# Yuer867/EMO-Disentanger

Hardware: AMD Instinct MI355X
Metric: train tokens/sec (+ AR gen tokens/sec in "gen"), stage2 Performer d512 L12 seq2048 (higher is better)
Workload: dtype bf16; 1 GPU; BASELINE configs[1]: stage2 Performer d_model=512 n_layer=12 n_head=8 favor_dims=128 seq=2048, B=64/GPU, dropout 0.1, omega redraw every_forward, fwd+bwd+allreduce+clip+Adam; global_batch=64, seq_len=2048, parallelism=dp1

## Files before the change

emo-disentanger_amd/csrc/emo_gemm_w128.hip:

```cpp
#include "emo_gemm_epi.h"

namespace {
constexpr int W_BM = 256, W_BN = 256, W_BK = 64;
constexpr int W_TILE = 256 * W_BK * 2;
constexpr int W_NA = 3, W_NB = 2;
constexpr int W_LDS = (W_NA + W_NB) * W_TILE;

__device__ __forceinline__ uint32_t w_lds_addr(const void* p) { return (uint32_t)(uintptr_t)(const __attribute__((address_space(3))) char*)p; }

__device__ __forceinline__ void w_dma2(const char* sbase, uint32_t o0, uint32_t o1, uint32_t lds_dst) {
    uint32_t keep;
    asm volatile("s_mov_b32 %0, m0\n\ts_mov_b32 m0, %4\n\ts_nop 0\n\tglobal_load_lds_dwordx4 %1, %3\n\ts_add_u32 m0, m0, 0x400\n\ts_nop 0\n\t"
                 "global_load_lds_dwordx4 %2, %3\n\ts_mov_b32 m0, %0"
                 : "=&s"(keep) : "v"(o0), "v"(o1), "s"(sbase), "s"(lds_dst) : "memory", "scc");
}
__device__ __forceinline__ void w_dma2_nt(const char* sbase, uint32_t o0, uint32_t o1, uint32_t lds_dst) {
    uint32_t keep;
    asm volatile("s_mov_b32 %0, m0\n\ts_mov_b32 m0, %4\n\ts_nop 0\n\tglobal_load_lds_dwordx4 %1, %3 nt\n\ts_add_u32 m0, m0, 0x400\n\ts_nop 0\n\t"
                 "global_load_lds_dwordx4 %2, %3 nt\n\ts_mov_b32 m0, %0"
                 : "=&s"(keep) : "v"(o0), "v"(o1), "s"(sbase), "s"(lds_dst) : "memory", "scc");
}
__device__ __forceinline__ void w_mma(f32x4& c, const bf16x8& a, const bf16x8& b) {
    asm volatile("v_mfma_f32_16x16x32_bf16 %0, %1, %2, %0" : "+a"(c) : "v"(a), "v"(b));
}
__device__ __forceinline__ void w_mma_v(f32x4& c, const bf16x8& a, const bf16x8& b) {
    asm volatile("s_nop 3\n\tv_mfma_f32_16x16x32_bf16 %0, %1, %2, %0" : "+v"(c) : "v"(a), "v"(b));
}
__device__ __forceinline__ void w_mma_drain() { asm volatile("s_nop 15\n\ts_nop 15" ::: "memory"); }
__device__ __forceinline__ void w_drop8(const DropCtx& d, uint64_t idx0, float (&v)[8]) {
    const uint32_t lo = (uint32_t)(idx0 >> 2), hi = (uint32_t)(idx0 >> 34) * 0x9E3779B1u;
#pragma unroll
    for (int q = 0; q < 2; ++q) {
        const uint32_t h = emo_drop_hash(d, (lo + q) ^ hi), h2 = emo_xs32(h);
        v[4 * q] *= (h & 0xFFFFu) >= d.thr16 ? d.scale : 0.f;
        v[4 * q + 1] *= (h >> 16) >= d.thr16 ? d.scale : 0.f;
        v[4 * q + 2] *= (h2 & 0xFFFFu) >= d.thr16 ? d.scale : 0.f;
        v[4 * q + 3] *= (h2 >> 16) >= d.thr16 ? d.scale : 0.f;
    }
}
template <int N> __device__ __forceinline__ void w_wait();
template <> __device__ __forceinline__ void w_wait<0>() { asm volatile("s_waitcnt vmcnt(0)" ::: "memory"); }
template <> __device__ __forceinline__ void w_wait<8>() { asm volatile("s_waitcnt vmcnt(8)" ::: "memory"); }
template <> __device__ __forceinline__ void w_wait<24>() { asm volatile("s_waitcnt vmcnt(24)" ::: "memory"); }

template <typename OutT>
__global__ __launch_bounds__(256, 1) void gemm_w128_kernel(const bf16_t* __restrict__ A, int64_t lda, const bf16_t* __restrict__ B, int64_t ldb,
                                                          OutT* __restrict__ C, int64_t M, int64_t N, int64_t K, EpiParams ep) {
    extern __shared__ __attribute__((aligned(16))) char smem[];
#ifdef EMO_DIAG
    const uint64_t dg_t0 = __builtin_readcyclecounter();
    uint64_t dg_sync = 0, dg_loop0 = 0, dg_loop1 = 0;
#endif
    const int tid = threadIdx.x, lane = tid & 63;
    const int wave = __builtin_amdgcn_readfirstlane(tid >> 6);
    const int wr = wave >> 1, wc = wave & 1;
    const int64_t tiles_n = N / W_BN, tiles_m = M / W_BM;
    const int64_t bid = blockIdx.x, xcd = bid & 7, local = bid >> 3;
    const int64_t tn = local % tiles_n, tm = (local / tiles_n) * 8 + xcd;
    if (tm >= tiles_m) return;
    const int64_t m0 = tm * W_BM, n0 = tn * W_BN;
    const int nk = (int)(K / W_BK);

    uint32_t offA[8], offB[8];
#pragma unroll
    for (int i = 0; i < 8; ++i) {
        const int r = (wave * 8 + i) * 8 + (lane >> 3);
        offA[i] = (uint32_t)((r * lda + ((lane & 7) ^ (r & 7)) * 8) * 2);
        offB[i] = (uint32_t)((r * ldb + ((lane & 7) ^ (((r >> 1) & 1) | (((r >> 3) & 3) << 1))) * 8) * 2);
    }
    const char* gA = (const char*)(A + m0 * lda);
    const char* gB = (const char*)(B + n0 * ldb);
    const uint32_t lds0 = __builtin_amdgcn_readfirstlane(w_lds_addr(smem));
    const uint32_t dstw = lds0 + wave * 8192;
    const uint32_t foA = (uint32_t)((lane & 15) * 128 + ((((lane >> 4)) ^ (lane & 7)) << 4)) + wr * 128 * 128;
    const uint32_t foB = (uint32_t)((8 * ((lane & 15) >> 2) + (lane & 3)) * 128 + (((lane >> 4) ^ (((lane >> 1) & 1) | (((lane >> 2) & 3) << 1))) << 4)) +
                         W_NA * W_TILE + wc * 128 * 128;

    f32x4 acc[8][8];
#pragma unroll
    for (int i = 0; i < 8; ++i)
#pragma unroll
        for (int j = 0; j < 8; ++j) acc[i][j] = (f32x4){0.f, 0.f, 0.f, 0.f};

    int sa_issue = 0, sb_issue = 0;
    int t_issueA = 0, t_issueB = 0;
    const bool a_nt = ep.a_nt != 0;
    auto issueA_part = [&](int g) {
        if (a_nt) w_dma2_nt(gA + (int64_t)t_issueA * (W_BK * 2), offA[2 * g], offA[2 * g + 1], dstw + sa_issue * W_TILE + g * 2048);
        else w_dma2(gA + (int64_t)t_issueA * (W_BK * 2), offA[2 * g], offA[2 * g + 1], dstw + sa_issue * W_TILE + g * 2048);
    };
    auto issueB_part = [&](int g) { w_dma2(gB + (int64_t)t_issueB * (W_BK * 2), offB[2 * g], offB[2 * g + 1], dstw + (W_NA + sb_issue) * W_TILE + g * 2048); };
    auto doneA = [&]() { ++t_issueA; sa_issue = sa_issue == W_NA - 1 ? 0 : sa_issue + 1; };
    auto doneB = [&]() { ++t_issueB; sb_issue ^= 1; };
#pragma unroll
    for (int s = 0; s < 5; ++s) {
        const bool isA = (s & 1) == 0;
#pragma unroll
        for (int g = 0; g < 4; ++g) { if (isA) issueA_part(g); else issueB_part(g); }
        if (isA) { doneA(); if (t_issueA > nk - 1) t_issueA = nk - 1; } else { doneB(); if (t_issueB > nk - 1) t_issueB = nk - 1; }
    }
    w_wait<24>();
    __builtin_amdgcn_s_barrier();
    asm volatile("" ::: "memory");

    bf16x8 fa[2][8], fb[2][8];
    int sa = 0, sb = 0;
    const char* ldsb = smem;
    auto rd = [&](int set, int q, uint32_t a_off, uint32_t b_off) {
        if (q < 8) fb[set][q] = *(const bf16x8*)(ldsb + b_off + (32 * (q >> 1) + 4 * (q & 1)) * 128);
        else fa[set][q - 8] = *(const bf16x8*)(ldsb + a_off + (q - 8) * 2048);
    };
    {
        const uint32_t a_off = foA, b_off = foB;
#pragma unroll
        for (int q = 0; q < 16; ++q) rd(0, q, a_off, b_off);
    }
    constexpr int RQ[9] = {0, 3, 6, 9, 12, 14, 16, 16, 16};
#ifdef EMO_DIAG
    dg_loop0 = __builtin_readcyclecounter();
#endif
    for (int t = 0; t < nk; ++t) {
        const uint32_t a_off = (foA + sa * W_TILE) ^ 64u, b_off = (foB + sb * W_TILE) ^ 64u;
#pragma unroll
        for (int i = 0; i < 8; ++i) {
#pragma unroll
            for (int q = RQ[i]; q < RQ[i + 1]; ++q) rd(1, q, a_off, b_off);
#pragma unroll
            for (int j = 0; j < 8; ++j) w_mma(acc[i][j], fb[0][j], fa[0][i]);
            __builtin_amdgcn_sched_barrier(0);
        }
#ifdef EMO_DIAG
        const uint64_t dg_s0 = __builtin_readcyclecounter();
#endif
        asm volatile("s_waitcnt lgkmcnt(0)" ::: "memory");
        w_wait<8>();
        __builtin_amdgcn_s_barrier();
        asm volatile("" ::: "memory");
#ifdef EMO_DIAG
        dg_sync += __builtin_readcyclecounter() - dg_s0;
#endif
        sa = sa == W_NA - 1 ? 0 : sa + 1;
        sb ^= 1;
        const uint32_t a_nx = foA + sa * W_TILE, b_nx = foB + sb * W_TILE;
#pragma unroll
        for (int i = 0; i < 8; ++i) {
#pragma unroll
            for (int q = RQ[i]; q < RQ[i + 1]; ++q) rd(0, q, a_nx, b_nx);
            if (i < 4) issueB_part(i); else issueA_part(i - 4);
#pragma unroll
            for (int j = 0; j < 8; ++j) w_mma(acc[i][j], fb[1][j], fa[1][i]);
            __builtin_amdgcn_sched_barrier(0);
        }
        doneB(); if (t_issueB > nk - 1) t_issueB = nk - 1;
        doneA(); if (t_issueA > nk - 1) t_issueA = nk - 1;
    }
#ifdef EMO_DIAG
    dg_loop1 = __builtin_readcyclecounter();
#endif
    w_wait<0>();
    w_mma_drain();
    const int ecol = 8 * (lane >> 4);
    {
        f32x4 bv[4][2];
#pragma unroll
        for (int h = 0; h < 4; ++h)
#pragma unroll
            for (int q = 0; q < 2; ++q) bv[h][q] = ep.bias ? *(const f32x4*)(ep.bias + n0 + wc * 128 + 32 * h + ecol + 4 * q) : (f32x4){0.f, 0.f, 0.f, 0.f};
        const OutT* rp = (const OutT*)ep.residual;
#pragma clang loop unroll(full)
        for (int i2 = 0; i2 < 4; ++i2) {
            bf16x8 res[2][4];
            if (rp) {
#pragma unroll
                for (int u = 0; u < 2; ++u)
#pragma unroll
                    for (int h = 0; h < 4; ++h)
                        res[u][h] = *(const bf16x8*)(rp + (m0 + wr * 128 + (2 * i2 + u) * 16 + (lane & 15)) * ep.ldc + n0 + wc * 128 + 32 * h + ecol);
            }
#pragma clang loop unroll(full)
            for (int u = 0; u < 2; ++u) {
                const int i = 2 * i2 + u;
                const int64_t m = m0 + wr * 128 + i * 16 + (lane & 15);
#pragma clang loop unroll(full)
                for (int h = 0; h < 4; ++h) {
                    const int64_t n = n0 + wc * 128 + 32 * h + ecol;
                    float v[8];
#pragma unroll
                    for (int r = 0; r < 4; ++r) { v[r] = acc[i][2 * h][r] + bv[h][0][r]; v[4 + r] = acc[i][2 * h + 1][r] + bv[h][1][r]; }
                    if (ep.drop.thr16) w_drop8(ep.drop, (uint64_t)(m * N + n), v);
                    if (rp) {
#pragma unroll
                        for (int r = 0; r < 8; ++r) v[r] += (float)res[u][h][r];
                    }
                    bf16x8 o;
#pragma unroll
                    for (int r = 0; r < 8; ++r) o[r] = (bf16_t)v[r];
                    if (ep.nt_store) __builtin_nontemporal_store(o, (bf16x8*)(C + m * ep.ldc + n));
                    else *(bf16x8*)(C + m * ep.ldc + n) = o;
                }
            }
        }
    }
#ifdef EMO_DIAG
    if (ep.ablate == 8 && ep.rln_stats && lane == 0) {
        unsigned long long* dg = (unsigned long long*)ep.rln_stats;
        const uint64_t t1 = __builtin_readcyclecounter();
        atomicAdd(dg + 0, (unsigned long long)(dg_loop0 - dg_t0));
        atomicAdd(dg + 1, (unsigned long long)(dg_loop1 - dg_loop0));
        atomicAdd(dg + 2, (unsigned long long)dg_sync);
        atomicAdd(dg + 3, (unsigned long long)(t1 - dg_loop1));
        atomicAdd(dg + 4, 1ull);
    }
#endif
}

__device__ __forceinline__ int w_swz_k(int k) { return (k & 3) | (((k >> 3) & 1) << 2); }

template <int RS>
__global__ __launch_bounds__(256, 1) void gemm_w128_tn_kernel(const bf16_t* __restrict__ A, int64_t lda, const bf16_t* __restrict__ B, int64_t ldb,
                                                             float* __restrict__ Cws, int64_t M, int64_t N, int64_t K, int64_t kps, float* __restrict__ a_rowsum, float* __restrict__ b_rowsum,
                                                             int full, int extra, int nt_mask, float* __restrict__ rs_ws) {
    extern __shared__ __attribute__((aligned(16))) char smem[];
    const int tid = threadIdx.x, lane = tid & 63;
    const int wave = __builtin_amdgcn_readfirstlane(tid >> 6);
    const int wr = wave >> 1, wc = wave & 1;
    const int64_t tiles_n = N / W_BN, ntile = (M / W_BM) * tiles_n;
    const int64_t bid = blockIdx.x, xcd = bid & 7, q = bid >> 3;
    int64_t split, t_id;
    if (q < (int64_t)full * ntile) { split = xcd * full + q / ntile; t_id = q % ntile; }
    else {
        const int64_t left = 32 - (int64_t)full * ntile, slot = xcd * left + (q - (int64_t)full * ntile);
        if (slot >= (int64_t)extra * ntile) return;
        split = 8 * full + slot / ntile;
        t_id = slot % ntile;
    }
    const int64_t tm = t_id / tiles_n, tn = t_id % tiles_n;
    const int64_t m0 = tm * W_BM, n0 = tn * W_BN;
    const int64_t kbeg = split * kps;
    const int64_t kend = (kbeg + kps < K) ? kbeg + kps : K;
    float* C = Cws + split * M * N;
    const int nk = kbeg < kend ? (int)((kend - kbeg) / W_BK) : 0;
    if (nk == 0) {
#pragma unroll 4
        for (int e = tid; e < 256 * 64; e += 256) *(f32x4*)(C + (m0 + (e >> 6)) * N + n0 + (e & 63) * 4) = (f32x4){0.f, 0.f, 0.f, 0.f};
        if (RS == 1 && rs_ws) rs_ws[(split * tiles_n + tn) * M + m0 + tid] = 0.f;
        if (RS == 2 && rs_ws) rs_ws[(split * (M / W_BM) + tm) * N + n0 + tid] = 0.f;
        return;
    }
    uint32_t offA[8], offB[8];
#pragma unroll
    for (int i = 0; i < 8; ++i) {
        const int J = wave * 8 + i, half = J >> 4, j = J & 15;
        const int k = j * 4 + (lane >> 4), p16 = lane & 15, g = (p16 >> 1) ^ w_swz_k(k);
        offA[i] = (uint32_t)((k * lda + half * 128 + (g * 2 + (p16 & 1)) * 8) * 2);
        offB[i] = (uint32_t)((k * ldb + half * 128 + (g * 2 + (p16 & 1)) * 8) * 2);
    }
    const char* gA = (const char*)(A + kbeg * lda + m0);
    const char* gB = (const char*)(B + kbeg * ldb + n0);
    const int64_t stepA = 64 * lda * 2, stepB = 64 * ldb * 2;
    const uint32_t lds0 = __builtin_amdgcn_readfirstlane(w_lds_addr(smem));
    const uint32_t dstw = lds0 + wave * 8192;
    const int li = lane & 15;
    const uint32_t fo = (uint32_t)((((lane >> 4) * 8 + (li >> 2)) * 256) | ((((li >> 2) & 3) | (((lane >> 4) & 1) << 2)) << 5) | ((li & 3) << 3));
    const uint32_t foA = fo + wr * 16384, foB = fo + W_NA * W_TILE + wc * 16384;

    f32x4 acc[8][8];
#pragma unroll
    for (int i = 0; i < 8; ++i)
#pragma unroll
        for (int j = 0; j < 8; ++j) acc[i][j] = (f32x4){0.f, 0.f, 0.f, 0.f};
    f32x4 rs[4];
#pragma unroll
    for (int u = 0; u < 4; ++u) rs[u] = (f32x4){0.f, 0.f, 0.f, 0.f};
    const bf16_t one_b = (bf16_t)1.f;
    bf16x8 ones = {one_b, one_b, one_b, one_b, one_b, one_b, one_b, one_b};
    asm volatile("" : "+v"(ones));
    const int rs_mod = RS == 2 ? (int)(M / W_BM) : (int)tiles_n, rs_me = RS == 2 ? (int)tm : (int)tn;
    int rs_phase = RS ? (int)((kbeg / W_BK) % rs_mod) : 0;

    int sa_issue = 0, sb_issue = 0, t_issueA = 0, t_issueB = 0;
    const bool a_nt = (nt_mask & 1) != 0, b_nt = (nt_mask & 2) != 0;
    auto issueA_part = [&](int g) {
        if (a_nt) w_dma2_nt(gA + (int64_t)t_issueA * stepA, offA[2 * g], offA[2 * g + 1], dstw + sa_issue * W_TILE + g * 2048);
        else w_dma2(gA + (int64_t)t_issueA * stepA, offA[2 * g], offA[2 * g + 1], dstw + sa_issue * W_TILE + g * 2048);
    };
    auto issueB_part = [&](int g) {
        if (b_nt) w_dma2_nt(gB + (int64_t)t_issueB * stepB, offB[2 * g], offB[2 * g + 1], dstw + (W_NA + sb_issue) * W_TILE + g * 2048);
        else w_dma2(gB + (int64_t)t_issueB * stepB, offB[2 * g], offB[2 * g + 1], dstw + (W_NA + sb_issue) * W_TILE + g * 2048);
    };
    auto doneA = [&]() { ++t_issueA; sa_issue = sa_issue == W_NA - 1 ? 0 : sa_issue + 1; if (t_issueA > nk - 1) t_issueA = nk - 1; };
    auto doneB = [&]() { ++t_issueB; sb_issue ^= 1; if (t_issueB > nk - 1) t_issueB = nk - 1; };
#pragma unroll
    for (int s = 0; s < 5; ++s) {
        const bool isA = (s & 1) == 0;
#pragma unroll
        for (int g = 0; g < 4; ++g) { if (isA) issueA_part(g); else issueB_part(g); }
        if (isA) doneA(); else doneB();
    }
    w_wait<24>();
    __builtin_amdgcn_s_barrier();
    asm volatile("" ::: "memory");

    bf16x8 fa[2][8], fb[2][8];
    int sa = 0, sb = 0;
    const char* ldsb = smem;
    auto rd1 = [&](uint32_t off) -> bf16x8 {
        bf16x8 v;
#pragma unroll
        for (int h = 0; h < 2; ++h) {
            const short4v t = __builtin_amdgcn_ds_read_tr16_b64_v4i16((__attribute__((address_space(3))) short4v*)(ldsb + off + h * 1024));
            const bf16x4 tb = __builtin_bit_cast(bf16x4, t);
            v[4 * h] = tb[0]; v[4 * h + 1] = tb[1]; v[4 * h + 2] = tb[2]; v[4 * h + 3] = tb[3];
        }
        return v;
    };
    auto rd = [&](int set, int q2, uint32_t a_off, uint32_t b_off, int ks8) {
        if (q2 < 8) fb[set][q2] = rd1((b_off ^ (uint32_t)(q2 << 5)) + ks8);
        else fa[set][q2 - 8] = rd1((a_off ^ (uint32_t)((q2 - 8) << 5)) + ks8);
    };
#pragma unroll
    for (int q2 = 0; q2 < 16; ++q2) rd(0, q2, foA, foB, 0);
    constexpr int RQ[9] = {0, 3, 6, 9, 12, 14, 16, 16, 16};
    for (int t = 0; t < nk; ++t) {
        const uint32_t a_off = foA + sa * W_TILE, b_off = foB + sb * W_TILE;
        const bool rs_on = RS && rs_phase == rs_me;
#pragma unroll
        for (int i = 0; i < 8; ++i) {
#pragma unroll
            for (int q2 = RQ[i]; q2 < RQ[i + 1]; ++q2) rd(1, q2, a_off, b_off, 8192);
#pragma unroll
            for (int j = 0; j < 8; ++j) w_mma(acc[i][j], fb[0][j], fa[0][i]);
            if (RS == 1 && rs_on && (i & 1) == wc) w_mma_v(rs[i >> 1], ones, fa[0][i]);
            if (RS == 2 && rs_on && (i & 1) == wr) w_mma_v(rs[i >> 1], fb[0][i], ones);
            __builtin_amdgcn_sched_barrier(0);
        }
        asm volatile("s_waitcnt lgkmcnt(0)" ::: "memory");
        w_wait<8>();
        __builtin_amdgcn_s_barrier();
        asm volatile("" ::: "memory");
        sa = sa == W_NA - 1 ? 0 : sa + 1;
        sb ^= 1;
        const uint32_t a_nx = foA + sa * W_TILE, b_nx = foB + sb * W_TILE;
#pragma unroll
        for (int i = 0; i < 8; ++i) {
#pragma unroll
            for (int q2 = RQ[i]; q2 < RQ[i + 1]; ++q2) rd(0, q2, a_nx, b_nx, 0);
            if (i < 4) issueB_part(i); else issueA_part(i - 4);
#pragma unroll
            for (int j = 0; j < 8; ++j) w_mma(acc[i][j], fb[1][j], fa[1][i]);
            if (RS == 1 && rs_on && (i & 1) == wc) w_mma_v(rs[i >> 1], ones, fa[1][i]);
            if (RS == 2 && rs_on && (i & 1) == wr) w_mma_v(rs[i >> 1], fb[1][i], ones);
            __builtin_amdgcn_sched_barrier(0);
        }
        doneB();
        doneA();
        if (RS) { if (++rs_phase == rs_mod) rs_phase = 0; }
    }
    w_wait<0>();
    w_mma_drain();
    if (RS == 1 && (lane >> 4) == 0) {
        float* dst = rs_ws ? rs_ws + (split * tiles_n + tn) * M : nullptr;
#pragma unroll
        for (int u = 0; u < 4; ++u) {
            const int64_t m = m0 + wr * 128 + (2 * u + wc) * 16 + lane;
            if (dst) dst[m] = rs[u][0]; else atomicAdd(a_rowsum + m, rs[u][0]);
        }
    }
    if (RS == 2 && (lane & 15) == 0) {
        float* dst = rs_ws ? rs_ws + (split * (M / W_BM) + tm) * N : nullptr;
#pragma unroll
        for (int u = 0; u < 4; ++u) {
            const int64_t n = n0 + wc * 128 + (2 * u + wr) * 16 + (lane >> 4) * 4;
            if (dst) *(f32x4*)(dst + n) = rs[u];
            else {
#pragma unroll
                for (int r = 0; r < 4; ++r) atomicAdd(b_rowsum + n + r, rs[u][r]);
            }
        }
    }
#pragma clang loop unroll(full)
    for (int i = 0; i < 8; ++i) {
        float* crow = C + (m0 + wr * 128 + i * 16 + (lane & 15)) * N + n0 + wc * 128 + (lane >> 4) * 4;
#pragma clang loop unroll(full)
        for (int j = 0; j < 8; ++j) *(f32x4*)(crow + j * 16) = acc[i][j];
    }
}
}

bool emo_gemm_w128_try(const bf16_t* A, int64_t lda, const bf16_t* B, int64_t ldb, void* C, int dtype_out, int64_t M, int64_t N, int64_t K,
                       const EpiParams& ep, hipStream_t st) {
    const char* e = getenv("EMO_GEMM_W128");
    const int mode = e ? atoi(e) : -1;
    if (mode == 0) return false;
    if ((M % W_BM) || (N % W_BN) || (K % W_BK) || K < 4 * W_BK || dtype_out != EMO_BF16) return false;
    if (mode < 0 && (K < 1024 || (M / W_BM) * (N / W_BN) < 256)) return false;
    if (ep.atomic || ep.accumulate || ep.ws_stride || ep.a_rowsum || ep.b_rowsum || ep.ln_c1 || ep.rln_x || ep.mask_out) return false;
    if (ep.aux_out || ep.mul_mode != EMO_MUL_NONE || ep.act != EMO_ACT_NONE) return false;
    if ((lda & 7) || (ldb & 7) || (ep.ldc & 7) || (((uintptr_t)A | (uintptr_t)B | (uintptr_t)C) & 15)) return false;
    if ((uint64_t)(256 * (lda > ldb ? lda : ldb) + 64) * 2 >= 0xFFFF0000ull) return false;
    const int64_t tiles_m = M / W_BM, tiles_n = N / W_BN;
    dim3 grid((unsigned)(((tiles_m + 7) / 8) * 8 * tiles_n));
    EpiParams ep2 = ep;
    { const char* e4 = getenv("EMO_W128_NT_STORE"); ep2.nt_store = e4 ? atoi(e4) : 0; }
    { const char* e3 = getenv("EMO_W128_A_NT"); ep2.a_nt = e3 ? atoi(e3) : 1; }
    auto k = gemm_w128_kernel<bf16_t>;
    static bool attr = false;
    if (!attr) { (void)hipFuncSetAttribute((const void*)k, hipFuncAttributeMaxDynamicSharedMemorySize, W_LDS); attr = true; }
    hipLaunchKernelGGL(k, grid, dim3(256), W_LDS, st, A, lda, B, ldb, (bf16_t*)C, M, N, K, ep2);
    return true;
}

static int64_t w_tn_plan(int64_t M, int64_t N, int64_t K, int& full, int& extra) {
    full = extra = 0;
    const char* e = getenv("EMO_GEMM_W128");
    if (e && atoi(e) == 0) return 0;
    const char* e2 = getenv("EMO_GEMM_W128_TN");
    if (e2 && atoi(e2) == 0) return 0;
    if ((M % W_BM) || (N % W_BN) || (K % W_BK)) return 0;
    const int64_t ntile = (M / W_BM) * (N / W_BN), nkt = K / W_BK;
    if (ntile > 32) return 0;
    int64_t f = 32 / ntile;
    if (f > 8) f = 8;
    int64_t x = f < 8 ? (8 * (32 - f * ntile)) / ntile : 0;
    if (e2 && atoi(e2) == 2) x = 0;
    int64_t min_kt = 16;
    { const char* e3 = getenv("EMO_W128_TN_MINKT"); if (e3 && atoi(e3) > 0) min_kt = atoi(e3); }
    while (nkt / (8 * f + x) < min_kt) {
        if (x) x = 0;
        else if (f > 1) --f;
        else return 0;
    }
    int64_t min_blk = 96;
    { const char* e4 = getenv("EMO_W128_TN_MINBLK"); if (e4 && atoi(e4) > 0) min_blk = atoi(e4); }
    if (ntile * (8 * f + x) < min_blk) return 0;
    full = (int)f;
    extra = (int)x;
    return 8 * f + x;
}
int64_t emo_gemm_w128_tn_splits(int64_t M, int64_t N, int64_t K) {
    int full, extra;
    return w_tn_plan(M, N, K, full, extra);
}

void emo_splitk_reduce_launch(const float* ws, int64_t stride, int splits, float* out, int64_t n4, int accumulate, hipStream_t st);
void emo_splitk_reduce_rs_launch(const float* ws, int64_t stride, int splits, float* out, int64_t n4, int accumulate, const float* rs_ws, int64_t rs_stride,
                                 int rs_parts, float* rs_out, hipStream_t st);
int64_t emo_gemm_w128_tn_rs_floats(int64_t M, int64_t N, int64_t splits) {
    const int64_t a = (N / W_BN) * M, b = (M / W_BM) * N;
    return splits * (a > b ? a : b);
}

bool emo_gemm_w128_tn_try(const bf16_t* A, int64_t lda, const bf16_t* B, int64_t ldb, float* C, int64_t ldc, int64_t M, int64_t N, int64_t K, int accumulate,
                          float* a_rowsum, float* b_rowsum, void* ws, int64_t ws_bytes, hipStream_t st) {
    int full, extra;
    const int64_t splits0 = w_tn_plan(M, N, K, full, extra);
    if (!splits0 || ldc != N || !ws || ((uintptr_t)ws & 15) || ws_bytes < splits0 * M * N * (int64_t)sizeof(float)) return false;
    if ((lda & 7) || (ldb & 7) || (((uintptr_t)A | (uintptr_t)B | (uintptr_t)C) & 15)) return false;
    if ((uint64_t)(64 * (lda > ldb ? lda : ldb) + 256) * 2 >= 0xFFFF0000ull) return false;
    const int64_t kps = ((K / W_BK + splits0 - 1) / splits0) * W_BK;
    const int64_t ntile = (M / W_BM) * (N / W_BN);
    dim3 grid(256);
    int nt_mask = 0;
    { const char* e3 = getenv("EMO_W128_TN_NT"); if (e3) nt_mask = atoi(e3); }
    float* rs_ws = nullptr;
    if ((a_rowsum || b_rowsum) && ws_bytes >= (splits0 * M * N + emo_gemm_w128_tn_rs_floats(M, N, splits0)) * (int64_t)sizeof(float) &&
        !(((uintptr_t)a_rowsum | (uintptr_t)b_rowsum) & 15))
        rs_ws = (float*)ws + splits0 * M * N;
#define W_TN_LAUNCH(RSv)                                                                                                                     \
    do {                                                                                                                                     \
        auto k = gemm_w128_tn_kernel<RSv>;                                                                                                   \
        static bool attr = false;                                                                                                            \
        if (!attr) { (void)hipFuncSetAttribute((const void*)k, hipFuncAttributeMaxDynamicSharedMemorySize, W_LDS); attr = true; }            \
        hipLaunchKernelGGL(k, grid, dim3(256), W_LDS, st, A, lda, B, ldb, (float*)ws, M, N, K, kps, a_rowsum, b_rowsum, full, extra, nt_mask, rs_ws); \
    } while (0)
    if (a_rowsum) W_TN_LAUNCH(1); else if (b_rowsum) W_TN_LAUNCH(2); else W_TN_LAUNCH(0);
#undef W_TN_LAUNCH
    if (rs_ws)
        emo_splitk_reduce_rs_launch((const float*)ws, M * N, (int)splits0, C, (M * N) >> 2, accumulate, rs_ws, a_rowsum ? M : N,
                                    (int)(splits0 * (a_rowsum ? N / W_BN : M / W_BM)), a_rowsum ? a_rowsum : b_rowsum, st);
    else
        emo_splitk_reduce_launch((const float*)ws, M * N, (int)splits0, C, (M * N) >> 2, accumulate, st);
    return true;
}
```

Baseline: 2.971 million tokens/s.

## Add 8-wave variant of split-K TN weight-gradient GEMM kernel

Adds a 512-thread (8-wave) version of the 256x256 split-K TN GEMM kernel. Each wave now owns a 128x64 sub-tile instead of 128x128, with per-wave DMA slices and wait counts adjusted to match. Higher-priority scheduling is set on the upper four waves. This becomes the default path, with an env var to fall back to the 4-wave kernel. The aim is more latency hiding and better MFMA/LDS overlap per CU. In exchange each wave does more LDS reads relative to its MFMA work.

```diff
diff --git a/emo-disentanger_amd/csrc/emo_gemm_w128.hip b/emo-disentanger_amd/csrc/emo_gemm_w128.hip
--- a/emo-disentanger_amd/csrc/emo_gemm_w128.hip
+++ b/emo-disentanger_amd/csrc/emo_gemm_w128.hip
@@ -40,7 +40,9 @@
 }
 template <int N> __device__ __forceinline__ void w_wait();
 template <> __device__ __forceinline__ void w_wait<0>() { asm volatile("s_waitcnt vmcnt(0)" ::: "memory"); }
+template <> __device__ __forceinline__ void w_wait<4>() { asm volatile("s_waitcnt vmcnt(4)" ::: "memory"); }
 template <> __device__ __forceinline__ void w_wait<8>() { asm volatile("s_waitcnt vmcnt(8)" ::: "memory"); }
+template <> __device__ __forceinline__ void w_wait<12>() { asm volatile("s_waitcnt vmcnt(12)" ::: "memory"); }
 template <> __device__ __forceinline__ void w_wait<24>() { asm volatile("s_waitcnt vmcnt(24)" ::: "memory"); }
 
 template <typename OutT>
@@ -384,6 +386,178 @@
 #pragma clang loop unroll(full)
         for (int j = 0; j < 8; ++j) *(f32x4*)(crow + j * 16) = acc[i][j];
     }
+}
+
+namespace w8 {
+template <int RS>
+__global__ __launch_bounds__(512, 1) void gemm_w128_tn_kernel(const bf16_t* __restrict__ A, int64_t lda, const bf16_t* __restrict__ B, int64_t ldb,
+                                                             float* __restrict__ Cws, int64_t M, int64_t N, int64_t K, int64_t kps, float* __restrict__ a_rowsum, float* __restrict__ b_rowsum,
+                                                             int full, int extra, int nt_mask, float* __restrict__ rs_ws) {
+    extern __shared__ __attribute__((aligned(16))) char smem[];
+    const int tid = threadIdx.x, lane = tid & 63;
+    const int wave = __builtin_amdgcn_readfirstlane(tid >> 6);
+    const int wm = wave >> 2, wn = wave & 3;
+    const int64_t tiles_n = N / W_BN, ntile = (M / W_BM) * tiles_n;
+    const int64_t bid = blockIdx.x, xcd = bid & 7, q = bid >> 3;
+    int64_t split, t_id;
+    if (q < (int64_t)full * ntile) { split = xcd * full + q / ntile; t_id = q % ntile; }
+    else {
+        const int64_t left = 32 - (int64_t)full * ntile, slot = xcd * left + (q - (int64_t)full * ntile);
+        if (slot >= (int64_t)extra * ntile) return;
+        split = 8 * full + slot / ntile;
+        t_id = slot % ntile;
+    }
+    const int64_t tm = t_id / tiles_n, tn = t_id % tiles_n;
+    const int64_t m0 = tm * W_BM, n0 = tn * W_BN;
+    const int64_t kbeg = split * kps;
+    const int64_t kend = (kbeg + kps < K) ? kbeg + kps : K;
+    float* C = Cws + split * M * N;
+    const int nk = kbeg < kend ? (int)((kend - kbeg) / W_BK) : 0;
+    if (nk == 0) {
+#pragma unroll 4
+        for (int e = tid; e < 256 * 64; e += 512) *(f32x4*)(C + (m0 + (e >> 6)) * N + n0 + (e & 63) * 4) = (f32x4){0.f, 0.f, 0.f, 0.f};
+        if (RS == 1 && rs_ws && tid < 256) rs_ws[(split * tiles_n + tn) * M + m0 + tid] = 0.f;
+        if (RS == 2 && rs_ws && tid < 256) rs_ws[(split * (M / W_BM) + tm) * N + n0 + tid] = 0.f;
+        return;
+    }
+    uint32_t offA[4], offB[4];
+#pragma unroll
+    for (int i = 0; i < 4; ++i) {
+        const int J = wave * 4 + i, half = J >> 4, j = J & 15;
+        const int k = j * 4 + (lane >> 4), p16 = lane & 15, g = (p16 >> 1) ^ w_swz_k(k);
+        offA[i] = (uint32_t)((k * lda + half * 128 + (g * 2 + (p16 & 1)) * 8) * 2);
+        offB[i] = (uint32_t)((k * ldb + half * 128 + (g * 2 + (p16 & 1)) * 8) * 2);
+    }
+    const char* gA = (const char*)(A + kbeg * lda + m0);
+    const char* gB = (const char*)(B + kbeg * ldb + n0);
+    const int64_t stepA = 64 * lda * 2, stepB = 64 * ldb * 2;
+    const uint32_t lds0 = __builtin_amdgcn_readfirstlane(w_lds_addr(smem));
+    const uint32_t dstw = lds0 + wave * 4096;
+    const int li = lane & 15;
+    const uint32_t fo = (uint32_t)((((lane >> 4) * 8 + (li >> 2)) * 256) | ((((li >> 2) & 3) | (((lane >> 4) & 1) << 2)) << 5) | ((li & 3) << 3));
+    const uint32_t foA = fo + wm * 16384, foB = (fo ^ (uint32_t)((wn & 1) << 7)) + W_NA * W_TILE + (wn >> 1) * 16384;
+
+    f32x4 acc[8][4];
+#pragma unroll
+    for (int i = 0; i < 8; ++i)
+#pragma unroll
+        for (int j = 0; j < 4; ++j) acc[i][j] = (f32x4){0.f, 0.f, 0.f, 0.f};
+    f32x4 rs[2];
+    rs[0] = rs[1] = (f32x4){0.f, 0.f, 0.f, 0.f};
+    const bf16_t one_b = (bf16_t)1.f;
+    bf16x8 ones = {one_b, one_b, one_b, one_b, one_b, one_b, one_b, one_b};
+    asm volatile("" : "+v"(ones));
+    const int rs_mod = RS == 2 ? (int)(M / W_BM) : (int)tiles_n, rs_me = RS == 2 ? (int)tm : (int)tn;
+    int rs_phase = RS ? (int)((kbeg / W_BK) % rs_mod) : 0;
+
+    int sa_issue = 0, sb_issue = 0, t_issueA = 0, t_issueB = 0;
+    const bool a_nt = (nt_mask & 1) != 0, b_nt = (nt_mask & 2) != 0;
+    auto issueA_part = [&](int g) {
+        if (a_nt) w_dma2_nt(gA + (int64_t)t_issueA * stepA, offA[2 * g], offA[2 * g + 1], dstw + sa_issue * W_TILE + g * 2048);
+        else w_dma2(gA + (int64_t)t_issueA * stepA, offA[2 * g], offA[2 * g + 1], dstw + sa_issue * W_TILE + g * 2048);
+    };
+    auto issueB_part = [&](int g) {
+        if (b_nt) w_dma2_nt(gB + (int64_t)t_issueB * stepB, offB[2 * g], offB[2 * g + 1], dstw + (W_NA + sb_issue) * W_TILE + g * 2048);
+        else w_dma2(gB + (int64_t)t_issueB * stepB, offB[2 * g], offB[2 * g + 1], dstw + (W_NA + sb_issue) * W_TILE + g * 2048);
+    };
+    auto doneA = [&]() { ++t_issueA; sa_issue = sa_issue == W_NA - 1 ? 0 : sa_issue + 1; if (t_issueA > nk - 1) t_issueA = nk - 1; };
+    auto doneB = [&]() { ++t_issueB; sb_issue ^= 1; if (t_issueB > nk - 1) t_issueB = nk - 1; };
+#pragma unroll
+    for (int s = 0; s < 5; ++s) {
+        const bool isA = (s & 1) == 0;
+#pragma unroll
+        for (int g = 0; g < 2; ++g) { if (isA) issueA_part(g); else issueB_part(g); }
+        if (isA) doneA(); else doneB();
+    }
+    w_wait<12>();
+    __builtin_amdgcn_s_barrier();
+    asm volatile("" ::: "memory");
+
+    bf16x8 fa[8], fb[2][4];
+    int sa = 0, sb = 0;
+    const char* ldsb = smem;
+    auto rd1 = [&](uint32_t off) -> bf16x8 {
+        bf16x8 v;
+#pragma unroll
+        for (int h = 0; h < 2; ++h) {
+            const short4v t = __builtin_amdgcn_ds_read_tr16_b64_v4i16((__attribute__((address_space(3))) short4v*)(ldsb + off + h * 1024));
+            const bf16x4 tb = __builtin_bit_cast(bf16x4, t);
+            v[4 * h] = tb[0]; v[4 * h + 1] = tb[1]; v[4 * h + 2] = tb[2]; v[4 * h + 3] = tb[3];
+        }
+        return v;
+    };
+    auto rdA = [&](int i, uint32_t a_off, int ks8) { fa[i] = rd1((a_off ^ (uint32_t)(i << 5)) + ks8); };
+    auto rdB = [&](int set, int j, uint32_t b_off, int ks8) { fb[set][j] = rd1((b_off ^ (uint32_t)(j << 5)) + ks8); };
+#pragma unroll
+    for (int j = 0; j < 4; ++j) rdB(0, j, foB, 0);
+#pragma unroll
+    for (int i = 0; i < 8; ++i) rdA(i, foA, 0);
+    if (wave >= 4) __builtin_amdgcn_s_setprio(1);
+    auto group = [&](int i, int set, bool rs_on) {
+#pragma unroll
+        for (int j = 0; j < 4; ++j) w_mma(acc[i][j], fb[set][j], fa[i]);
+        if (RS == 1 && rs_on && (i & 3) == wn) w_mma_v(rs[i >> 2], ones, fa[i]);
+        if (RS == 2 && rs_on && i < 4 && (i & 1) == wm) w_mma_v(rs[i >> 1], fb[set][i], ones);
+    };
+    for (int t = 0; t < nk; ++t) {
+        const uint32_t a_off = foA + sa * W_TILE, b_off = foB + sb * W_TILE;
+        const bool rs_on = RS && rs_phase == rs_me;
+#pragma unroll
+        for (int i = 0; i < 8; ++i) {
+            group(i, 0, rs_on);
+            if (i < 2) { rdB(1, 2 * i, b_off, 8192); rdB(1, 2 * i + 1, b_off, 8192); }
+            rdA(i, a_off, 8192);
+            __builtin_amdgcn_sched_barrier(0);
+        }
+        asm volatile("s_waitcnt lgkmcnt(0)" ::: "memory");
+        w_wait<4>();
+        __builtin_amdgcn_s_barrier();
+        asm volatile("" ::: "memory");
+        sa = sa == W_NA - 1 ? 0 : sa + 1;
+        sb ^= 1;
+        const uint32_t a_nx = foA + sa * W_TILE, b_nx = foB + sb * W_TILE;
+#pragma unroll
+        for (int i = 0; i < 8; ++i) {
+            group(i, 1, rs_on);
+            if (i < 2) { rdB(0, 2 * i, b_nx, 0); rdB(0, 2 * i + 1, b_nx, 0); }
+            rdA(i, a_nx, 0);
+            if ((i & 1) == 0) { if (i < 4) issueB_part(i >> 1); else issueA_part((i - 4) >> 1); }
+            __builtin_amdgcn_sched_barrier(0);
+        }
+        doneB();
+        doneA();
+        if (RS) { if (++rs_phase == rs_mod) rs_phase = 0; }
+    }
+    if (wave >= 4) __builtin_amdgcn_s_setprio(0);
+    w_wait<0>();
+    w_mma_drain();
+    if (RS == 1 && (lane >> 4) == 0) {
+        float* dst = rs_ws ? rs_ws + (split * tiles_n + tn) * M : nullptr;
+#pragma unroll
+        for (int u = 0; u < 2; ++u) {
+            const int64_t m = m0 + wm * 128 + (4 * u + wn) * 16 + lane;
+            if (dst) dst[m] = rs[u][0]; else atomicAdd(a_rowsum + m, rs[u][0]);
+        }
+    }
+    if (RS == 2 && (lane & 15) == 0) {
+        float* dst = rs_ws ? rs_ws + (split * (M / W_BM) + tm) * N : nullptr;
+#pragma unroll
+        for (int u = 0; u < 2; ++u) {
+            const int64_t n = n0 + wn * 64 + (2 * u + wm) * 16 + (lane >> 4) * 4;
+            if (dst) *(f32x4*)(dst + n) = rs[u];
+            else {
+#pragma unroll
+                for (int r = 0; r < 4; ++r) atomicAdd(b_rowsum + n + r, rs[u][r]);
+            }
+        }
+    }
+#pragma clang loop unroll(full)
+    for (int i = 0; i < 8; ++i) {
+        float* crow = C + (m0 + wm * 128 + i * 16 + (lane & 15)) * N + n0 + wn * 64 + (lane >> 4) * 4;
+#pragma clang loop unroll(full)
+        for (int j = 0; j < 4; ++j) *(f32x4*)(crow + j * 16) = acc[i][j];
+    }
+}
 }
 }
 
@@ -410,6 +584,13 @@
     return true;
 }
 
+template <auto KERN> static void w_lds_attr() {
+    static bool done[64] = {};
+    int dev = 0;
+    if (hipGetDevice(&dev) != hipSuccess || dev < 0 || dev >= 64) dev = 0;
+    if (!done[dev]) { (void)hipFuncSetAttribute((const void*)KERN, hipFuncAttributeMaxDynamicSharedMemorySize, W_LDS); done[dev] = true; }
+}
+
 static int64_t w_tn_plan(int64_t M, int64_t N, int64_t K, int& full, int& extra) {
     full = extra = 0;
     const char* e = getenv("EMO_GEMM_W128");
@@ -466,14 +647,19 @@
     if ((a_rowsum || b_rowsum) && ws_bytes >= (splits0 * M * N + emo_gemm_w128_tn_rs_floats(M, N, splits0)) * (int64_t)sizeof(float) &&
         !(((uintptr_t)a_rowsum | (uintptr_t)b_rowsum) & 15))
         rs_ws = (float*)ws + splits0 * M * N;
-#define W_TN_LAUNCH(RSv)                                                                                                                     \
-    do {                                                                                                                                     \
-        auto k = gemm_w128_tn_kernel<RSv>;                                                                                                   \
-        static bool attr = false;                                                                                                            \
-        if (!attr) { (void)hipFuncSetAttribute((const void*)k, hipFuncAttributeMaxDynamicSharedMemorySize, W_LDS); attr = true; }            \
-        hipLaunchKernelGGL(k, grid, dim3(256), W_LDS, st, A, lda, B, ldb, (float*)ws, M, N, K, kps, a_rowsum, b_rowsum, full, extra, nt_mask, rs_ws); \
+    const char* e5 = getenv("EMO_W128_TN_WAVES");
+    const bool eight = !(e5 && atoi(e5) == 4);
+#define W_TN_LAUNCH(KERN)                                                                                                                        \
+    do {                                                                                                                                         \
+        w_lds_attr<KERN>();                                                                                                                      \
+        hipLaunchKernelGGL(KERN, grid, dim3(eight ? 512 : 256), W_LDS, st, A, lda, B, ldb, (float*)ws, M, N, K, kps, a_rowsum, b_rowsum, full, extra, \
+                           nt_mask, rs_ws);                                                                                                      \
     } while (0)
-    if (a_rowsum) W_TN_LAUNCH(1); else if (b_rowsum) W_TN_LAUNCH(2); else W_TN_LAUNCH(0);
+    if (eight) {
+        if (a_rowsum) W_TN_LAUNCH(w8::gemm_w128_tn_kernel<1>); else if (b_rowsum) W_TN_LAUNCH(w8::gemm_w128_tn_kernel<2>); else W_TN_LAUNCH(w8::gemm_w128_tn_kernel<0>);
+    } else {
+        if (a_rowsum) W_TN_LAUNCH(gemm_w128_tn_kernel<1>); else if (b_rowsum) W_TN_LAUNCH(gemm_w128_tn_kernel<2>); else W_TN_LAUNCH(gemm_w128_tn_kernel<0>);
+    }
 #undef W_TN_LAUNCH
     if (rs_ws)
         emo_splitk_reduce_rs_launch((const float*)ws, M * N, (int)splits0, C, (M * N) >> 2, accumulate, rs_ws, a_rowsum ? M : N,
```

Result: no change. 2.987 million tokens/s, median of 6 (+0.6%).
